# BEAMRobotics/beam_slam

Hardware: AMD Instinct MI355X
Metric: LM iterations/sec + ms/graph-solve, 200KF x 50k-landmark VIO window (higher is better)
Workload: dtype f64; 1 GPU; C2: 200-keyframe x 50000-landmark VIO window; n_obs=400690, n_imu_factors=199, solver_options=vio.yaml:7-17 (<= 10 iterations, tolerances 1.5e-7), max_solver_time lifted, parallelism=single GPU, n_ranks_seen=1

## Files before the change

beam_slam_amd/capi.py:

```python
import ctypes as C

import numpy as np

OK = 0
ERR_INVALID, ERR_DEVICE, ERR_UNSUPPORTED, ERR_NUMERIC = -1, -2, -3, -4

MANIFOLD_EUCLIDEAN, MANIFOLD_QUAT_RIGHT = 0, 1
LOSS_TRIVIAL, LOSS_CAUCHY, LOSS_HUBER = 0, 1, 2

F_REPROJ = 0
F_REPROJ_ONLINE_CALIB = 1
F_IMU_DELTA = 2
F_IMU_PRIOR = 3
F_RELPOSE_EXT = 4
F_RELPOSE = 5
F_ABSPOSE = 6
F_ABS_VEC3 = 7
F_REL_VEC3 = 8
F_GRAVITY = 9
F_IDP_REPROJ = 10
F_IDP_REPROJ_UNARY = 11
F_UNICYCLE = 12
F_NUM_TYPES = 13

# ... 53 lines not shown
        ("iteration", C.c_int32),
        ("step_is_valid", C.c_int32),
        ("step_is_successful", C.c_int32),
        ("reserved0", C.c_int32),
        ("cost", C.c_double),
        ("cost_change", C.c_double),
        ("gradient_max_norm", C.c_double),
        ("gradient_norm", C.c_double),
        ("step_norm", C.c_double),
        ("relative_decrease", C.c_double),
        ("trust_region_radius", C.c_double),
        ("model_cost_change", C.c_double),
    ]


class Camera(C.Structure):
    _fields_ = [
        ("fx", C.c_double), ("fy", C.c_double), ("cx", C.c_double), ("cy", C.c_double),
        ("R_cam_baselink", C.c_double * 9),
        ("t_cam_baselink", C.c_double * 3),
    ]


SYMBOLS = [
    "nidx", "nconst", "nres", "options_default", "options_vio", "create", "create_error", "destroy",
    "last_error", "abi_version", "clear", "set_blocks", "set_values", "set_cameras", "add_factors", "add_factors_indirect", "sync_factors_indirect",
    "add_marginal",
    "finalize", "solve", "get_blocks", "reset_values", "num_iterations_recorded", "get_iteration",
    "evaluate", "num_residuals", "num_parameters_tangent", "tangent_offset", "covariance", "marginalize", "get_marginal",
    "reprojection_errors", "preintegrate", "triangulate", "time_reproj_jacobian_ms", "reproj_jacobian_bytes", "dense_solve", "plan_info",
    "profile_step", "time_eval_ms", "eval_bytes", "bsr_info", "covariance_joint", "update_marginal", "solve_batch", "batch_stats", "set_plan_preference",
    "covariance_requests", "localize_frames", "num_factorizations", "essential_ransac", "absolute_pose_ransac",
    "relative_pose_ransac", "inertial_alignment", "register_scans", "register_scans_error", "backsub_tangent_table",
    "scan_context_describe", "scan_context_match", "scan_context_error",
]

_dp = C.POINTER(C.c_double)
_ip = C.POINTER(C.c_int32)
_bp = C.POINTER(C.c_uint8)

RANSAC_OK, RANSAC_TOO_FEW, RANSAC_NO_MODEL = 0, 1, 2
RANSAC_MAX_MATCHES = 65536
ESSENTIAL_RANSAC_ARGTYPES = [C.c_void_p, C.c_int32, _ip, _dp, _dp, _dp, C.c_double, C.c_double, C.c_int32, C.c_uint64, _bp, _dp, _ip, _ip,
                             _ip, _ip]
ABSOLUTE_POSE_RANSAC_ARGTYPES = [C.c_void_p, C.c_int32, _ip, _dp, _dp, _ip, C.c_double, C.c_double, C.c_int32, C.c_uint64, C.c_int32, _bp,
                                 _dp, _dp, _dp, _ip, _ip, _ip, _ip]
RELATIVE_POSE_RANSAC_ARGTYPES = [C.c_void_p, C.c_int32, _ip, _dp, _dp, _ip, C.c_double, C.c_double, C.c_int32, C.c_uint64, C.c_int32,
                                 C.c_double, C.c_double, _bp, _dp, _dp, _dp, _dp, _bp, _dp, _ip, _ip, _ip, _ip, _ip]
ALIGN_OK, ALIGN_TOO_FEW_FRAMES, ALIGN_BAD_IMU, ALIGN_NOT_EXCITED, ALIGN_RANK_DEFICIENT, ALIGN_SCALE_REJECTED = 0, 1, 2, 3, 4, 5
ALIGN_MIN_EXCITATION, ALIGN_SCALE_MIN, ALIGN_SCALE_MAX, ALIGN_RANK_TOL = 0.25, 0.02, 1.0, 1e-10
INERTIAL_ALIGNMENT_ARGTYPES = [C.c_int, C.c_int32, _ip, _dp, _dp, _dp, _ip, _dp, _dp, _dp, C.c_int32, C.c_double, C.c_int32, C.c_double,
                               C.c_double, C.c_double, _dp, _dp, _dp, _dp, _ip, _dp, _dp, _dp, _dp, _ip]
ICP_MAX_ITERATIONS, ICP_TRANSFORM, ICP_ABS_MSE, ICP_REL_MSE, ICP_TOO_FEW_CORRESPONDENCES = 1, 2, 3, 4, 5
ICP_MAX_CELLS, ICP_MAX_ITER = 1 << 22, 1000
ICP_DEFAULTS = dict(max_corr=1.0, max_iter=50, t_eps=1e-8, fit_eps=1e-2, rotation_threshold=0.99999, rel_mse_eps=1e-5)
REGISTER_SCANS_ARGTYPES = [C.c_int, C.c_int32, _ip, _dp, _ip, _dp, _dp, C.c_double, C.c_int32, C.c_double, C.c_double, C.c_double,
                           C.c_double, _dp, _dp, _dp, _ip, _ip, _ip]
SC_RINGS, SC_SECTORS, SC_MAX_CANDIDATES, SC_MAX_TREE_CANDIDATES, SC_MAX_SCAN_POINTS = 20, 60, 65536, 64, 65535 * 4096
SC_DEFAULTS = dict(lidar_height=2.0, max_radius=80.0, n_tree_candidates=10, search_ratio=0.1, dist_thres=0.3)
SCAN_CONTEXT_DESCRIBE_ARGTYPES = [C.c_int, C.c_int32, _ip, _dp, C.c_int32, _ip, _ip, _dp, C.c_double, C.c_double, _dp, _dp, _dp, _ip]
SCAN_CONTEXT_MATCH_ARGTYPES = [C.c_int, C.c_int32, _ip, _dp, _ip, _dp, C.c_int32, C.c_double, C.c_double, _ip, _dp, _ip, _dp, _dp, _ip]


def _ptr(a, typ):
    return None if a is None else a.ctypes.data_as(typ)


# ... 297 lines not shown
```

beam_slam_amd/csrc/bsgpu_api.cpp:

```cpp
#include <thread>

#include "bsgpu_ctx.h"
#include "bsgpu_env.h"

using namespace bsg;

namespace bsg {
int api_exception(bsgpu_ctx* c) noexcept {
  int code = BSGPU_ERR_INVALID;
  const char* what = "unexpected exception";
  try { throw; }
  catch (const std::bad_alloc&) { code = BSGPU_ERR_DEVICE; what = "out of host memory"; }
  catch (const std::exception& e) { what = e.what(); try { if (c) c->err = std::string("internal error: ") + what; } catch (...) {} return code; }
  catch (...) {}
  try { if (c) c->err = what; } catch (...) {}
  return code;
}
thread_local std::string g_create_error;
int invalidate_keep_values(bsgpu_ctx* c) {
  if (c->finalized && c->d_x && !c->h_x.empty()) {
    HIPCHK(c, hipSetDevice(c->device));
    HIPCHK(c, hipStreamSynchronize(c->stream));
    HIPCHK(c, hipMemcpy(c->h_x.data(), c->d_x, sizeof(double) * c->h_x.size(), hipMemcpyDeviceToHost));
  }
// ... 959 lines not shown
  eval_all(c, c->d_x, true, SC_COST_X);
  (void)hipEventRecord(e0, c->stream);
  for (int i = 0; i < reps; ++i) eval_all(c, c->d_x, true, SC_COST_X);
  (void)hipEventRecord(e1, c->stream);
  if (hipEventSynchronize(e1) != hipSuccess) return -1.0;
  float ms = 0.f;
  (void)hipEventElapsedTime(&ms, e0, e1);
  (void)hipEventDestroy(e0); (void)hipEventDestroy(e1);
  c->spec_J = false;
  return (double)ms / reps;
}
int64_t bsgpu_eval_bytes(const bsgpu_ctx* c) {
  if (!c) return -1;
  static const struct { int idx, consts, res, jcols; } L[BSGPU_F_NUM_TYPES] = {
      {4, 3, 2, 9}, {6, 3, 2, 9}, {10, 287, 15, 30}, {5, 241, 15, 15}, {6, 43, 6, 12}, {4, 43, 6, 12}, {2, 43, 6, 6}, {1, 12, 3, 3},
      {2, 12, 3, 6}, {1, 7, 2, 3}, {6, 6, 2, 13}, {4, 6, 2, 7}, {10, 226, 15, 30}};
  int64_t b = (int64_t)c->vis.n * (c->vis.ja == kJACompact ? 152 : 200) + (int64_t)c->h_x.size() * 8;
  for (int t = 2; t < BSGPU_F_NUM_TYPES && t < kNumInternal; ++t)
    b += (int64_t)c->small[t].n * (4 * L[t].idx + 8 * (L[t].consts + L[t].res + L[t].res * L[t].jcols));
  return b;
}
int bsgpu_bsr_info(bsgpu_ctx* c, int32_t* block_rows, int32_t* nnz_blocks) try {
  if (!c) return BSGPU_ERR_INVALID;
  const int rc = finalize(c);
  if (rc != BSGPU_OK) return rc;
  if (block_rows) *block_rows = c->use_pcg ? c->nbr : 0;
  if (nnz_blocks) *nnz_blocks = c->use_pcg ? c->nblk : 0;
  return BSGPU_OK;
} catch (...) { return api_exception(c); }
int bsgpu_profile_step(bsgpu_ctx* c, const bsgpu_options* o, int32_t reps, double* ms_out, double* work_out) try {
  if (!c) return BSGPU_ERR_INVALID;
  if (!o || !ms_out || reps <= 0) return fail(c, BSGPU_ERR_INVALID, "profile_step: bad argument");
  return profile_step(c, *o, reps, ms_out, work_out);
} catch (...) { return api_exception(c); }
int64_t bsgpu_reproj_jacobian_bytes(const bsgpu_ctx* c) {
  if (!c) return -1;
  return (int64_t)c->vis.n * (c->vis.ja == kJACompact ? 152 : 200) + (int64_t)c->h_x.size() * 8;
}

int bsgpu_dense_solve(int device, int32_t n, const double* A, const double* b, double* x, int32_t max_chains, double* ms_out) try {
  if (n <= 0 || !A || !b || !x) return BSGPU_ERR_INVALID;
  if (hipSetDevice(device) != hipSuccess) return BSGPU_ERR_DEVICE;
  chol_prepare();
  const int T = (n + 63) / 64;
  std::vector<uint8_t> adj((size_t)T * T, 0);
  for (int i = 0; i < n; ++i) for (int j = 0; j < n; ++j) if (A[(size_t)i * n + j] != 0.0) adj[(size_t)(i / 64) * T + j / 64] = 1;
  DensePlan P;
  P.build(n, adj, std::max(1, (int)max_chains), 1, env_shared());
  const int npad = P.npad;
  std::vector<double> hS((size_t)npad * npad, 0.0);
  for (int i = 0; i < n; ++i) for (int j = 0; j < n; ++j) hS[(size_t)P.spos(i) * npad + P.spos(j)] = A[(size_t)i * n + j];
  for (int j = 0; j < n; ++j) hS[(size_t)P.rhs_row * npad + P.spos(j)] = b[j];
  std::vector<uint8_t> real(npad, 0);
  for (int j = 0; j < n; ++j) real[P.spos(j)] = 1;
  for (int i = 0; i < npad; ++i) if (!real[i]) hS[(size_t)i * npad + i] = 1.0;
  double *dS = nullptr, *dLp = nullptr, *dV = nullptr, *dy = nullptr, *dscal = nullptr;
  int *dnreal = nullptr, *drows = nullptr;
  PanelDesc *dpan = nullptr, *dsep = nullptr;
  int *dpot2 = nullptr, *dcb = nullptr, *dce = nullptr, *dsync = nullptr, *dfsync = nullptr, *dtot = nullptr;
  double* dW = nullptr;
  FusedTask* dft = nullptr;
  const bool fused = env_chol_fused() && !P.ftasks.empty();
  hipStream_t s;
  if (hipStreamCreate(&s) != hipSuccess) return BSGPU_ERR_DEVICE;
  auto up = [](const void* src, size_t bytes, void** dst) {
    if (hipMalloc(dst, bytes ? bytes : 8) != hipSuccess) return false;
// ... 74 lines not shown
```

beam_slam_amd/csrc/bsgpu_ctx.h:

```cpp
#pragma once
#include <hip/hip_runtime.h>

#include <algorithm>
#include <chrono>
#include <cmath>
#include <cstdio>
#include <cstdlib>
#include <cstring>
#include <limits>
#include <map>
#include <mutex>
#include <string>
#include <vector>

#include "../../include/bsgpu.h"
#include "bsgpu_internal.h"
#include "dense_plan.h"


namespace bsg {


struct TypeInfo { int nidx, nvar, nconst, m; int amb[10]; };
constexpr int T_REPROJ_DENSE = BSGPU_F_NUM_TYPES;
// ... 118 lines not shown
  double* d_small_part[kNumInternal] = {nullptr};
  double* d_small_part_cand[kNumInternal] = {nullptr};
  double* d_small_part_mcc[kNumInternal] = {nullptr};
  SmallGroup* d_small_groups = nullptr;
  SmallGroup small_factorwise[kNumInternal];
  int n_sa_seg = 0;
  int *d_sa_seg_start = nullptr, *d_sa_seg_ra = nullptr, *d_sa_seg_rb = nullptr;
  int2* d_sa_contrib = nullptr;
  int n_asm_grp = 0;
  AsmGroup* d_asm_grp = nullptr;
  ReduceEntry* d_reduce = nullptr;
  int n_reduce = 0;
  double* d_part_upd = nullptr;
  double* d_gpart = nullptr;
  int n_gpart = 0;
  int n_part_upd = 0;
  int n_upd_blocks = 0;
  bool pre_cleared = false;
  bool upd_in_mcc = false;
  int* d_upd_blocks = nullptr;
  int* d_lm_xoff = nullptr;
  double *d_S = nullptr, *d_grad = nullptr, *d_hdiag = nullptr, *d_scale = nullptr, *d_dcl = nullptr;
  double *d_delta = nullptr, *d_y = nullptr, *d_scal = nullptr, *d_part = nullptr;
  double* h_scal = nullptr;
  double* h_scal_dev = nullptr;
  int dim_model = -1, dim_model_age = 0, dim_model_npose = -1;
  int plan_pref = 0;
  bool spec_dev = false;
  unsigned dec_count = 0;
  double* d_dec = nullptr;
  double spec_lm_radius = 0.0;
  bool spec_cand_arrays = false;
  bool reduce_carried = false;
  bool xpart_stale = false;
  bool spec_dirty = false;
  bool scal_mirrored = false;
  DensePlan plan;
  std::vector<uint8_t> tile_adj;
  int *d_dpos = nullptr, *d_inat = nullptr;
  int *d_nreal = nullptr, *d_rows_flat = nullptr;
  PanelDesc* d_panels = nullptr;
  int *d_bs_desc_chain = nullptr, *d_rows_flat_chain = nullptr, *d_bs_upd = nullptr, *d_bs_upd_rows = nullptr;
  int *d_bs_chain_group = nullptr, *d_bs_grp_nchains = nullptr, *d_bs_grp_nitems = nullptr, *d_bs_items4 = nullptr, *d_bs_tile_updated = nullptr, *d_bs_sync = nullptr, *d_bs_order = nullptr;
  int *d_bs_desc = nullptr, *d_chain_begin = nullptr, *d_chain_end = nullptr, *d_tile_sync = nullptr, *d_touched = nullptr;
  int n_touched = 0;
  int* d_tile_tot = nullptr;
  FusedTask* d_ftasks = nullptr;
  FusedTask* d_ftasks_rows = nullptr; int n_ftasks_rows = 0;
  FusedTask* d_ftasks_bulk = nullptr; int* d_tile_tot_bulk = nullptr; int n_ftasks_bulk = 0;
  FusedTask* d_ftasks_plain = nullptr; int* d_tile_tot_plain = nullptr; int n_ftasks_plain = 0;
  int* d_fsync = nullptr;
  double* d_Vinv = nullptr;
  double* d_Winv = nullptr;
  double* d_Lp = nullptr;
  double* d_ytan = nullptr;
  std::vector<bsgpu_iteration> iters;
  hipGraphExec_t g_first = nullptr, g_accept = nullptr, g_reject = nullptr;
  bool graphs_tried = false, graphs_ok = false, use_graphs = true;
  bsgpu_options graph_opts{};
  double* h_radius = nullptr;
  double* h_pcg = nullptr;
  hipEvent_t pcg_ev[2] = {nullptr, nullptr};
  double* h_pcg_lazy = nullptr;
  bool pcg_check_pending = false;
  int pcg_verdicts_seen = 0;
  hipEvent_t ev_reduce = nullptr;
// ... 99 lines not shown
  std::memcpy(d.R, hc.R_cam_baselink, sizeof(d.R));
  std::memcpy(d.t, hc.t_cam_baselink, sizeof(d.t));
  return d;
}
inline std::vector<DevCamera> dev_cameras(const bsgpu_ctx* c) {
  std::vector<DevCamera> cams;
  cams.reserve(c->cams.size());
  for (const bsgpu_camera& hc : c->cams) cams.push_back(to_dev_camera(hc));
  return cams;
}

#define HIPCHK(c, call)                                                                         \
  do { hipError_t e_ = (call); if (e_ != hipSuccess) return fail(c, BSGPU_ERR_DEVICE, std::string(#call) + ": " + hipGetErrorString(e_)); } while (0)

int materialize_mirror(bsgpu_ctx* c);
int finalize(bsgpu_ctx* c);
int build_bsr(bsgpu_ctx* c);
int build_spcg(bsgpu_ctx* c);
int solve(bsgpu_ctx* c, const bsgpu_options& o, bsgpu_summary& sum);
int check_strategy(bsgpu_ctx* c, const bsgpu_options& o);
void enqueue_fixed_cost(bsgpu_ctx* c, hipStream_t s);
void eval_all(bsgpu_ctx* c, const double* x, bool with_J, int slot, const ReduceRide* red = nullptr);
void assemble(bsgpu_ctx* c, const bsgpu_options& o, double radius, bool new_J, bool first, bool gradient_only = false, bool factor_follows = false,
              const ReduceRide* red = nullptr );
void final_reduce(bsgpu_ctx* c);
int fetch_scalars(bsgpu_ctx* c);
int ensure_vis_src(bsgpu_ctx* c);
void dense_factor(hipStream_t s, const DensePlan& P, const DenseDev& D, double* S, double* scal);
void dense_backsolve(hipStream_t s, const DensePlan& P, const DenseDev& D, double* S, double* y, const int* iperm = nullptr,
                     int n_pose = 0, double* y_tan = nullptr, double* delta = nullptr);
void dense_factor_solve(hipStream_t s, const DensePlan& P, const DenseDev& D, double* S, double* y, double* scal, const int* iperm = nullptr,
                        int n_pose = 0, double* y_tan = nullptr, double* delta = nullptr);
int profile_step(bsgpu_ctx* c, const bsgpu_options& o, int reps, double* ms_out, double* work_out);
bool batch_covers(bsgpu_ctx* c, const bsgpu_options& o);
void batch_stats(int64_t* windows, int64_t* rounds);
bool solve_batched(bsgpu_ctx* const* ctxs, const int* idx, int m, const bsgpu_options* o, int options_stride, bsgpu_summary* s, int* rc);
void batch_forget(const bsgpu_ctx* c);

}
```

beam_slam_amd/csrc/bsgpu_internal.h:

```cpp
#pragma once
#include <hip/hip_runtime.h>
#include <stdint.h>

#include <functional>
#include <cstring>
#include <vector>

#include "dense_plan.h"

struct bsgpu_options;

namespace bsg {

struct DevCamera {
  double fx, fy, cx, cy;
  double R[9];
  double t[3];
};
struct DevLoss {
  int kind;
  int pad;
  double a;
};

// ... 316 lines not shown
void batchargs_small_assemble_seg(BatchArgTable& t, const SmallGroup* groups_dev, int n_seg, const int* seg_start, const int* seg_ra, const int* seg_rb, const int2* contrib,
                                  double* S, int ld, int rhs_row, double* grad, double* hdiag, const int* perm, const SmallGroupSet* fw, int n_fw_units, int n_grp,
                                  const AsmGroup* grp);
void launch_small_assemble_seg_batch(hipStream_t s, const BatchArgTable& t, const BatchDyn* dyn, int list, int n);
bool batchargs_small_mcc(BatchArgTable& t, const SmallGroup* groups, double* const* parts, int n_groups, const double* delta, const UpdateRide* upd, const ZeroStep* zero);
void launch_small_mcc_batch(hipStream_t s, const BatchArgTable& t, const BatchDyn* dyn, int list, int n);
void batchargs_zero_tiles_multi(BatchArgTable& t, const ZeroStep* zs);
void launch_zero_tiles_multi_batch(hipStream_t s, const BatchArgTable& t, const BatchDyn* dyn, int list, int n);
struct MargDev;
bool batchargs_marg_eval(BatchArgTable& t, const MargDev* m, const double* x, double* cost_part);
void launch_marg_eval_batch(hipStream_t s, const BatchArgTable& t, const BatchDyn* dyn, int list, int n, bool with_J);
void batchargs_marg_assemble(BatchArgTable& t, const MargDev* m, double* S, int ld, int rhs_row, double* grad, double* hdiag, const int* perm);
void launch_marg_assemble_batch(hipStream_t s, const BatchArgTable& t, const BatchDyn* dyn, int list, int n);
void batchargs_marg_mcc(BatchArgTable& t, const MargDev* m, const double* delta_tan, double* part);
void launch_marg_mcc_batch(hipStream_t s, const BatchArgTable& t, const BatchDyn* dyn, int list, int n);
struct IdpElim;
void batchargs_idp_landmark(BatchArgTable& t, BatchArgTable& t_view, const IdpElim& e, const SmallGroup& g, int jacobi, double lm_lo, double lm_hi, double* scale, double* dcl, double* grad);
void launch_idp_landmark_batch(hipStream_t s, const BatchArgTable& t, const BatchArgTable& t_view, const BatchDyn* dyn, int list, int n);
void batchargs_idp_pairs(BatchArgTable& t, const IdpElim& e, const SmallGroup& g, double* S, int ld, int rhs_row, double* grad, double* hdiag, const int* perm);
void launch_idp_pairs_batch(hipStream_t s, const BatchArgTable& t, const BatchDyn* dyn, int list, int n);
void batchargs_idp_backsub(BatchArgTable& t, const IdpElim& e, const double* y_pose, double* delta);
void launch_idp_backsub_batch(hipStream_t s, const BatchArgTable& t, const BatchDyn* dyn, int list, int n);
int batchargs_backsolve(BatchArgTable* tabs, const DensePlan& P, const DenseDev& D, double* y, const int* iperm, int n_pose, double* y_tan, double* delta);
void launch_backsolve_batch(hipStream_t s, const BatchArgTable* tabs, const BatchDyn* dyn, const int* n_in_form);
void launch_landmark(hipStream_t s, const Visual& v, int n_pose, const double* radius_ptr, int compute_scale,
                     int compute_dcl, int jacobi, double lm_lo, double lm_hi, double* scale, double* dcl,
                     double* grad, const ZeroStep* zero = nullptr, double radius_val = 0.0, const ReduceRide* red = nullptr );
void launch_pairs(hipStream_t s, const Visual& v, double* S, int ld, int rhs_row, double* grad, double* hdiag, const int* perm,
                  bool grad_only, const SmallGroupSet* small = nullptr, int n_small_units = 0, GoWord go = GoWord());
bool band_available();
void launch_pairs_band(hipStream_t s, const Visual& v, double* S, int ld, int rhs_row, double* grad, double* hdiag, const int* perm,
                       bool grad_only, const SmallGroupSet* small = nullptr, int n_small_units = 0, bool lower_only = false ,
                       GoWord go = GoWord());
int small_assemble_first_set(const SmallGroup* groups, int n_groups, SmallGroupSet* set, int* n_taken);
void launch_small_assemble_set(hipStream_t s, const SmallGroup* groups, int n_groups, double* S, int ld, int rhs_row, double* grad,
                               double* hdiag, const int* perm);
constexpr int kAsmGroupMax = 24;
struct AsmGroup {
  int type, count, m, nv;
  int toff[6];
  int te;
  int pad;
  const double* J;
  const double* r;
  int fac[kAsmGroupMax];
};
bool launch_small_assemble_seg(hipStream_t s, const SmallGroup* groups_dev, int n_seg, const int* seg_start, const int* seg_ra, const int* seg_rb,
                               const int2* contrib, double* S, int ld, int rhs_row, double* grad, double* hdiag, const int* perm,
                               const SmallGroupSet* fw = nullptr, int n_fw_units = 0, int n_grp = 0, const AsmGroup* grp = nullptr,
                               const MargDev* marg = nullptr, const ReduceRide* red = nullptr ,
                               bool* red_carried = nullptr);
void launch_pose_diag(hipStream_t s, int n_pose, double* S, int ld, const double* hdiag, const double* radius_ptr,
                      int compute_scale, int compute_dcl, int jacobi, double lm_lo, double lm_hi, double* scale,
                      double* dcl, int npad, const int* iperm, double radius_val = 0.0 );
void launch_grad_norms(hipStream_t s, int nb, const int* blk_xoff, const int* blk_toff, const unsigned char* blk_size,
                       const unsigned char* blk_manifold, const double* x, const double* grad, double* gpart );
void launch_grad_norms_pose_diag(hipStream_t s, int nb, const int* blk_xoff, const int* blk_toff, const unsigned char* blk_size,
                                 const unsigned char* blk_manifold, const double* x, const double* grad, double* gpart, int n_pose, double* S,
                                 int ld, const double* hdiag, const double* radius_ptr, int compute_scale, int compute_dcl, int jacobi,
                                 double lm_lo, double lm_hi, double* scale, double* dcl, int npad, const int* iperm, double radius_val = 0.0);
struct PanelDesc;
struct FusedTask;
void launch_chol_fused(hipStream_t s, double* S, double* Lp, int ld, const FusedTask* tasks_dev, int n_tasks, const int* tile_tot_dev, const int* nreal_dev,
                       double* Vinv, double* scal, int* sync_dev, double* Winv, int rhs_rows ,
                       const LmDiag& diag = LmDiag(), const GradNormRide& gn = GradNormRide(),
                       bool diag_tasks_in_list = false );
// ... 182 lines not shown
```

beam_slam_amd/csrc/bsgpu_solve.cpp:

```cpp
#include <atomic>

#include <thread>

#include "bsgpu_ctx.h"
#include "bsgpu_env.h"
#include "lm_state.h"

namespace bsg {

void assemble_pcg(bsgpu_ctx* c, const bsgpu_options& o, double radius, bool new_J, bool first) {
  hipStream_t s = c->stream;
  launch_zero4(s, c->d_val, (int64_t)c->nblk * 9, c->d_rhs, c->n_pose, c->d_grad, c->n_pose, c->d_hdiag, c->n_pose);
  for (int t = 2; t < kNumInternal; ++t) launch_bsr_assemble(s, c->small[t], c->d_slots[t], c->d_val);
  launch_bsr_assemble_seg(s, c->d_small_groups, c->n_bsr_seg, c->d_bsr_seg_start, c->d_bsr_seg_slot, c->d_bsr_seg_row, c->d_bsr_contrib, c->d_val, c->d_rhs,
                          c->d_grad, c->d_hdiag);
  launch_bsr_finish_diag(s, c->nbr, c->d_diag_slot, c->d_pair_slot, c->d_val, c->d_hdiag, radius, first ? 1 : 0, new_J ? 1 : 0, o.jacobi_scaling,
                         o.min_lm_diagonal, o.max_lm_diagonal, c->d_scale, c->d_dcl, c->d_Minv);
  if (new_J) {
    launch_grad_norms(s, c->nb, c->d_blk_xoff, c->d_blk_toff, c->d_blk_size, c->d_blk_manifold, c->d_x, c->d_grad, c->d_gpart);
  }
}

static std::atomic<int> g_pcg_persistent_in_flight{0};
void pcg_solve(bsgpu_ctx* c, const bsgpu_options& o) {
// ... 196 lines not shown
  for (size_t i = 0; i < c->marg.size(); ++i) {
    const auto& mc = c->marg[i];
    if (mc.active && (int)i != marg_done) launch_marg_eval(s, mc.dev, x, with_J, cand ? mc.part_cand : mc.part);
  }
  if (with_J) phase_mark(c, BSGPU_PHASE_EVAL_OTHER);
}
bool reduce_can_ride(const bsgpu_ctx* c) {
  static const bool by_event = env_scalars_event(), off = env_reduce_launch();
  return !off && !by_event && !c->use_graphs && !c->use_pcg && !c->prof_events && c->h_scal_dev != nullptr && c->d_reduce_counter != nullptr && c->n_reduce > 0;
}
bool reduce_rides(const bsgpu_ctx* c) {
  static const bool by_event = env_scalars_event(), off = env_reduce_launch();
  static const int merge_mode = env_eval_merge();
  const bool imu_pair = c->small[BSGPU_F_IMU_DELTA].n + c->small[BSGPU_F_IMU_PRIOR].n > 0;
  const bool carrier = imu_pair && merge_mode >= 2 && (c->vis.n > 0 || c->small[BSGPU_F_RELPOSE_EXT].n > 0 || c->small[BSGPU_F_RELPOSE].n > 0);
  return !off && !by_event && !c->use_graphs && !c->use_pcg && !c->prof_events && carrier && c->h_scal_dev != nullptr && c->d_reduce_counter != nullptr &&
         c->n_reduce > 0;
}
void final_reduce(bsgpu_ctx* c) {
  static const bool by_event = env_scalars_event();
  const bool stamp = !c->use_graphs && !by_event && c->h_scal_dev != nullptr && c->d_reduce_counter != nullptr && c->n_reduce > 0;
  if (stamp) c->reduce_seq += 1.0;
  launch_final_reduce(c->stream, c->d_reduce, c->n_reduce, SC_GRAD_NORM2 + 1, c->d_scal, c->h_scal_dev, stamp ? c->d_reduce_counter : nullptr, c->reduce_seq);
  c->scal_mirrored = c->h_scal_dev != nullptr && c->n_reduce > 0;
  c->seq_pending = stamp;
  if (stamp) { c->ev_reduce_pending = false; return; }
  if (c->use_graphs) { c->ev_reduce_pending = false; return; }
  if (!c->ev_reduce && hipEventCreateWithFlags(&c->ev_reduce, hipEventDisableTiming) != hipSuccess) { c->ev_reduce = nullptr; (void)hipGetLastError(); }
  c->ev_reduce_pending = c->scal_mirrored && c->ev_reduce && hipEventRecord(c->ev_reduce, c->stream) == hipSuccess;
}

void assemble(bsgpu_ctx* c, const bsgpu_options& o, double radius, bool new_J, bool first, bool gradient_only, bool factor_follows, const ReduceRide* red) {
  c->reduce_carried = false;
  if (c->use_pcg) { assemble_pcg(c, o, radius, new_J, first); return; }
  hipStream_t s = c->stream;
  ZeroStep zs;
  zs.S = c->d_S; zs.ld = c->npad; zs.tiles = c->d_touched; zs.n_tiles = c->n_touched;
  zs.a = c->d_grad; zs.na = c->n_pose; zs.b = c->d_hdiag; zs.nb = c->n_pose;
  zs.c = new_J ? c->d_scal + SC_GRAD_MAX : c->d_scal + SC_CHOL_FAIL; zs.nc = new_J ? 3 : 1;
  zs.radius_slot = c->use_graphs ? nullptr : c->d_scal + SC_RADIUS; zs.radius = radius;
  const bool dev_decides = red != nullptr && red->lmd.on && red->dec != nullptr && c->vis.n_lm > 0;
  GoWord go;
  if (dev_decides) { zs.radius_slot = nullptr; go.p = red->dec; }
  const bool merged = c->vis.n_lm > 0 && !c->use_graphs;
  const bool cleared = c->pre_cleared && !merged && !c->use_graphs;
  c->pre_cleared = false;
  if (!merged && !cleared) launch_zero_tiles_multi(s, zs.S, zs.ld, zs.tiles, zs.n_tiles, zs.a, zs.na, zs.b, zs.nb, zs.c, zs.nc, zs.radius_slot, zs.radius);
  c->scal_mirrored = false;
  const bool red_in_lm = red != nullptr && c->vis.n_lm > 0;
  if (red_in_lm) zs.nc = 0;
  launch_landmark(s, c->vis, c->n_pose, merged ? nullptr : c->d_scal + SC_RADIUS, first ? 1 : 0, new_J ? 1 : 0, o.jacobi_scaling, o.min_lm_diagonal,
                  o.max_lm_diagonal, c->d_scale, c->d_dcl, c->d_grad, merged ? &zs : nullptr, radius, red_in_lm ? red : nullptr);
  if (red_in_lm) c->reduce_carried = true;
  launch_idp_landmark(s, c->idp, c->small[BSGPU_F_IDP_REPROJ], c->use_graphs ? c->d_scal + SC_RADIUS : nullptr, radius, first ? 1 : 0, new_J ? 1 : 0,
                      o.jacobi_scaling, o.min_lm_diagonal, o.max_lm_diagonal, c->d_scale, c->d_dcl, c->d_grad);
  launch_idp_pairs(s, c->idp, c->small[BSGPU_F_IDP_REPROJ], c->d_S, c->npad, c->plan.rhs_row, c->d_grad, c->d_hdiag, c->d_dpos, gradient_only);
  phase_mark(c, BSGPU_PHASE_LANDMARK);
  int marg_done = -1;
  {
    SmallGroupSet set;
    int taken = 0, units = 0;
    const bool band = c->vis.n_band_units > 0;
    if (c->vis.n_seg > 0 || band) units = small_assemble_first_set(c->small_factorwise + 2, kNumInternal - 2, &set, &taken);
    if (units == 0) taken = 0;
    const bool lower_only = factor_follows && !gradient_only && !c->use_spcg && !c->use_pcg && c->dense_ok && c->d_ftasks && c->d_fsync && c->d_tile_tot && c->d_Winv;
    if (band) launch_pairs_band(s, c->vis, c->d_S, c->npad, c->plan.rhs_row, c->d_grad, c->d_hdiag, c->d_dpos, gradient_only, units > 0 ? &set : nullptr, units, lower_only, go);
    launch_pairs(s, c->vis, c->d_S, c->npad, c->plan.rhs_row, c->d_grad, c->d_hdiag, c->d_dpos, gradient_only, (units > 0 && !band) ? &set : nullptr, band ? 0 : units, go);
    if (c->calib.on) launch_calib_border(s, c->vis, c->calib, c->d_S, c->npad, c->plan.rhs_row, c->d_grad, c->d_hdiag, c->d_dpos, gradient_only);
// ... 274 lines not shown
    c->spec_J = false;
    c->prof_events = ev.data() + (size_t)r * ne;
    (void)hipEventRecord(c->prof_events[0], c->stream);
    enqueue_step(c, o, STEP_ACCEPT, radius);
    c->prof_events = nullptr;
  }
  HIPCHK(c, hipStreamSynchronize(c->stream));
  c->scal_mirrored = false; c->ev_reduce_pending = false; c->spec_J = false;
  for (int p = 0; p < BSGPU_PHASE_NUM; ++p) ms_out[p] = 0.0;
  for (int r = 0; r < reps; ++r)
    for (int p = 0; p < BSGPU_PHASE_NUM; ++p) {
      float ms = 0.f;
      (void)hipEventElapsedTime(&ms, ev[(size_t)r * ne + p], ev[(size_t)r * ne + p + 1]);
      ms_out[p] += (double)ms / reps;
    }
  for (auto& e : ev) (void)hipEventDestroy(e);
  if (work_out) {
    const double n = (double)c->vis.n, ne_ = (double)c->vis.n_elim, nl = (double)c->vis.n_lm, nent = (double)c->vis.n_ent;
    for (int p = 0; p < BSGPU_PHASE_NUM; ++p) work_out[p] = 0.0;
    const double ja_b = 8.0 * c->vis.ja;
    work_out[BSGPU_PHASE_EVAL_REPROJ] = n * (104.0 + ja_b) + 8.0 * (double)c->h_x.size();
    const double cr = c->vis.no_cr ? 0.0 : 64.0;
    work_out[BSGPU_PHASE_LANDMARK] = ne_ * (48.0 + 16.0 + cr) + nl * (72.0 + 24.0 + 48.0 + 4.0) + 32768.0 * (double)c->n_touched + 16.0 * (double)c->n_pose;
    work_out[BSGPU_PHASE_PAIRS] = ne_ * (ja_b + (c->vis.no_cr ? 48.0 : 64.0) + (c->vis.n_band_units > 0 ? 16.0 : 0.0)) + nent * 8.0 + (c->vis.no_cr ? nl * 72.0 : 0.0);
    work_out[BSGPU_PHASE_FACTOR] = c->plan.fused_flops;
    work_out[BSGPU_PHASE_BACKSUB] = n * (ja_b + 48.0 + 16.0) + ne_ * cr + nl * 72.0;
    work_out[BSGPU_PHASE_CANDIDATE] = n * 40.0 + 3.0 * 8.0 * (double)c->h_x.size();
  }
  HIPCHK(c, hipMemcpyAsync(c->d_x, c->d_x0, sizeof(double) * c->h_x.size(), hipMemcpyDeviceToDevice, c->stream));
  HIPCHK(c, hipStreamSynchronize(c->stream));
  return BSGPU_OK;
}

bool same_graph_options(const bsgpu_options& a, const bsgpu_options& b) {
  return a.jacobi_scaling == b.jacobi_scaling && a.min_lm_diagonal == b.min_lm_diagonal && a.max_lm_diagonal == b.max_lm_diagonal &&
         a.linear_solver_type == b.linear_solver_type;
}

void build_graphs(bsgpu_ctx* c, const bsgpu_options& o) {
  if (c->graphs_tried && same_graph_options(o, c->graph_opts)) return;
  c->destroy_graphs();
  c->graphs_tried = true;
  c->graph_opts = o;
  if (!c->use_graphs || c->use_pcg || c->use_spcg) return;
  hipGraphExec_t* execs[3] = {&c->g_first, &c->g_accept, &c->g_reject};
  for (int kind = 0; kind < 3; ++kind) {
    hipGraph_t graph = nullptr;
    if (hipStreamBeginCapture(c->stream, hipStreamCaptureModeThreadLocal) != hipSuccess) { (void)hipGetLastError(); return; }
    enqueue_step(c, o, kind, 1.0);
    if (hipStreamEndCapture(c->stream, &graph) != hipSuccess || !graph) { (void)hipGetLastError(); c->destroy_graphs(); c->graphs_tried = true; return; }
    const hipError_t e = hipGraphInstantiate(execs[kind], graph, nullptr, nullptr, 0);
    (void)hipGraphDestroy(graph);
    if (e != hipSuccess) { (void)hipGetLastError(); c->destroy_graphs(); c->graphs_tried = true; return; }
  }
  c->graphs_ok = true;
  if (env_timing()) fprintf(stderr, "[bsgpu] LM step captured as hipGraphs\n");
}

void run_step(bsgpu_ctx* c, const bsgpu_options& o, int kind, double radius, bool gradient_only = false, double radius_ahead = 0.0, const LmDecide* lmd = nullptr) {
  if (c->use_graphs) {
    *c->h_radius = radius;
    (void)hipMemcpyAsync(c->d_scal + SC_RADIUS, c->h_radius, sizeof(double), hipMemcpyHostToDevice, c->stream);
  }
  if (c->graphs_ok && !gradient_only) {
    hipGraphExec_t g = kind == STEP_FIRST ? c->g_first : kind == STEP_ACCEPT ? c->g_accept : c->g_reject;
    if (hipGraphLaunch(g, c->stream) == hipSuccess) return;
// ... 311 lines not shown
```

beam_slam_amd/gpu.py:

```python
import ctypes
import os

from . import capi

_HERE = os.path.dirname(os.path.abspath(__file__))
LIB_PATH = os.path.join(_HERE, "csrc", "libbsgpu.so")
_LIB = None


class GpuLibraryMissing(RuntimeError):
    pass


def lib():
    global _LIB
    if _LIB is None:
        if not os.path.exists(LIB_PATH):
            raise GpuLibraryMissing(
                f"{LIB_PATH} is missing: build it with `python -c 'import __graft_entry__ as g; g.build()'` "
                "(hipcc --offload-arch=gfx950).  beam_slam_amd has no CPU fallback.")
        _LIB = ctypes.CDLL(LIB_PATH)
        _LIB.bsgpu_time_reproj_jacobian_ms.restype = ctypes.c_double
        _LIB.bsgpu_time_reproj_jacobian_ms.argtypes = [ctypes.c_void_p, ctypes.c_int32]
        _LIB.bsgpu_time_eval_ms.restype = ctypes.c_double
# ... 294 lines not shown

    def eval_bytes(self):
        return lib().bsgpu_eval_bytes(self._ctx)

    def bsr_info(self):
        a, b = ctypes.c_int32(0), ctypes.c_int32(0)
        self._chk(lib().bsgpu_bsr_info(ctypes.c_void_p(self._ctx), ctypes.byref(a), ctypes.byref(b)))
        return a.value, b.value

    PHASES = ("eval_reproj", "eval_other", "landmark", "pairs", "assemble_other", "factor", "backsolve", "backsub", "candidate")

    def profile_step(self, options=None, reps=10):
        import numpy as np
        opt = options if options is not None else self.options_default()
        ms, work = np.zeros(len(self.PHASES)), np.zeros(len(self.PHASES))
        fn = lib().bsgpu_profile_step
        fn.argtypes = [ctypes.c_void_p, ctypes.c_void_p, ctypes.c_int32, ctypes.c_void_p, ctypes.c_void_p]
        self._chk(fn(self._ctx, ctypes.byref(opt), int(reps), ms.ctypes.data, work.ctypes.data))
        return {name: (float(ms[i]), float(work[i])) for i, name in enumerate(self.PHASES)}

    def set_plan_preference(self, throughput):
        fn = lib().bsgpu_set_plan_preference
        fn.argtypes = [ctypes.c_void_p, ctypes.c_int32]
        self._chk(fn(self._ctx, 1 if throughput else 0))

    def plan_info(self):
        a, b, c = ctypes.c_int32(0), ctypes.c_int32(0), ctypes.c_int32(0)
        self.finalize()
        lib().bsgpu_plan_info(ctypes.c_void_p(self._ctx), ctypes.byref(a), ctypes.byref(b), ctypes.byref(c))
        return a.value, b.value, c.value

    def reproj_jacobian_bytes(self):
        return lib().bsgpu_reproj_jacobian_bytes(self._ctx)
```

include/bsgpu.h:

```cpp
#ifndef BSGPU_H_
#define BSGPU_H_

#include <stdint.h>

#ifdef __cplusplus
extern "C" {
#endif

#define BSGPU_ABI_VERSION 1

enum {
  BSGPU_OK = 0,
  BSGPU_ERR_INVALID = -1,
  BSGPU_ERR_DEVICE = -2,
  BSGPU_ERR_UNSUPPORTED = -3,
  BSGPU_ERR_NUMERIC = -4
};

enum {
  BSGPU_MANIFOLD_EUCLIDEAN = 0,
  BSGPU_MANIFOLD_QUAT_RIGHT = 1
};

enum {
// ... 228 lines not shown
                           double* E, int32_t* n_inliers, int32_t* n_iters, int32_t* best_sample, int32_t* status);

int bsgpu_absolute_pose_ransac(bsgpu_ctx* ctx, int32_t n_frames, const int32_t* obs_start, const double* pixels,
                               const double* points, const int32_t* camera, double prob, double threshold_px,
                               int32_t max_iters, uint64_t seed, int32_t truncate_pixels, uint8_t* mask,
                               double* q_out, double* p_out, double* T_cam_world, int32_t* n_inliers,
                               int32_t* n_iters, int32_t* best_sample, int32_t* status);

int bsgpu_relative_pose_ransac(bsgpu_ctx* ctx, int32_t n_sets, const int32_t* match_start, const double* px_first,
                               const double* px_last, const int32_t* camera, double prob, double threshold_px,
                               int32_t max_iters, uint64_t seed, int32_t truncate_pixels, double validate_px,
                               double min_inlier_ratio, uint8_t* mask, double* T_last_first, double* q_out, double* p_out,
                               double* points, uint8_t* valid_mask, double* inlier_ratio, int32_t* pair_valid,
                               int32_t* n_inliers, int32_t* n_iters, int32_t* best_sample, int32_t* status);

double bsgpu_time_reproj_jacobian_ms(bsgpu_ctx* ctx, int32_t reps);
double bsgpu_time_eval_ms(bsgpu_ctx* ctx, int32_t reps);
int64_t bsgpu_eval_bytes(const bsgpu_ctx* ctx);
int bsgpu_bsr_info(bsgpu_ctx* ctx, int32_t* block_rows, int32_t* nnz_blocks);
int64_t bsgpu_reproj_jacobian_bytes(const bsgpu_ctx* ctx);
enum {
  BSGPU_PHASE_EVAL_REPROJ = 0,
  BSGPU_PHASE_EVAL_OTHER = 1,
  BSGPU_PHASE_LANDMARK = 2,
  BSGPU_PHASE_PAIRS = 3,
  BSGPU_PHASE_ASSEMBLE_OTHER = 4,
  BSGPU_PHASE_FACTOR = 5,
  BSGPU_PHASE_BACKSOLVE = 6,
  BSGPU_PHASE_BACKSUB = 7,
  BSGPU_PHASE_CANDIDATE = 8,
  BSGPU_PHASE_NUM = 9
};
int bsgpu_profile_step(bsgpu_ctx* ctx, const bsgpu_options* options, int32_t reps, double* ms_out, double* work_out);

int bsgpu_dense_solve(int device, int32_t n, const double* A, const double* b, double* x,
                      int32_t max_chains, double* ms_out);
int bsgpu_plan_info(const bsgpu_ctx* ctx, int32_t* n_chains, int32_t* n_steps, int32_t* n_tiles);
enum { BSGPU_PLAN_LATENCY = 0, BSGPU_PLAN_THROUGHPUT = 1 };
int bsgpu_set_plan_preference(bsgpu_ctx* ctx, int32_t preference);

#ifdef __cplusplus
}
#endif
#endif
```

Measured before the change: 3837 LM iterations/s.

## Add a dedicated visual gradient kernel for gradient-only assembly

Adds a gradient-only assembly path that skips building the Schur complement. A new kernel accumulates landmark and camera-pose gradients from the reprojection Jacobians, using LDS atomics per camera and riding the small factors in the same launch. The path only runs when graphs are off and several other conditions hold, and a new gradient_step API exercises it. In the normal LM solve with graphs enabled the new path is likely skipped, so it may not change timed iterations.

```diff
diff --git a/beam_slam_amd/capi.py b/beam_slam_amd/capi.py
--- a/beam_slam_amd/capi.py
+++ b/beam_slam_amd/capi.py
@@ -109,7 +109,7 @@
     "profile_step", "time_eval_ms", "eval_bytes", "bsr_info", "covariance_joint", "update_marginal", "solve_batch", "batch_stats", "set_plan_preference",
     "covariance_requests", "localize_frames", "num_factorizations", "essential_ransac", "absolute_pose_ransac",
     "relative_pose_ransac", "inertial_alignment", "register_scans", "register_scans_error", "backsub_tangent_table",
-    "scan_context_describe", "scan_context_match", "scan_context_error",
+    "scan_context_describe", "scan_context_match", "scan_context_error", "gradient_step",
 ]
 
 _dp = C.POINTER(C.c_double)
diff --git a/beam_slam_amd/csrc/bsgpu_api.cpp b/beam_slam_amd/csrc/bsgpu_api.cpp
--- a/beam_slam_amd/csrc/bsgpu_api.cpp
+++ b/beam_slam_amd/csrc/bsgpu_api.cpp
@@ -1015,6 +1015,11 @@
   if (!c) return BSGPU_ERR_INVALID;
   if (!o || !ms_out || reps <= 0) return fail(c, BSGPU_ERR_INVALID, "profile_step: bad argument");
   return profile_step(c, *o, reps, ms_out, work_out);
+} catch (...) { return api_exception(c); }
+int bsgpu_gradient_step(bsgpu_ctx* c, const bsgpu_options* o, double* gradient, int32_t* used_gradient_launch) try {
+  if (!c) return BSGPU_ERR_INVALID;
+  if (!o || !gradient) return fail(c, BSGPU_ERR_INVALID, "gradient_step: bad argument");
+  return gradient_step(c, *o, gradient, used_gradient_launch);
 } catch (...) { return api_exception(c); }
 int64_t bsgpu_reproj_jacobian_bytes(const bsgpu_ctx* c) {
   if (!c) return -1;
diff --git a/beam_slam_amd/csrc/bsgpu_ctx.h b/beam_slam_amd/csrc/bsgpu_ctx.h
--- a/beam_slam_amd/csrc/bsgpu_ctx.h
+++ b/beam_slam_amd/csrc/bsgpu_ctx.h
@@ -174,6 +174,7 @@
   double spec_lm_radius = 0.0;
   bool spec_cand_arrays = false;
   bool reduce_carried = false;
+  bool grad_launch_used = false;
   bool xpart_stale = false;
   bool spec_dirty = false;
   bool scal_mirrored = false;
@@ -339,6 +340,7 @@
 void dense_factor_solve(hipStream_t s, const DensePlan& P, const DenseDev& D, double* S, double* y, double* scal, const int* iperm = nullptr,
                         int n_pose = 0, double* y_tan = nullptr, double* delta = nullptr);
 int profile_step(bsgpu_ctx* c, const bsgpu_options& o, int reps, double* ms_out, double* work_out);
+int gradient_step(bsgpu_ctx* c, const bsgpu_options& o, double* gradient, int32_t* used_gradient_launch);
 bool batch_covers(bsgpu_ctx* c, const bsgpu_options& o);
 void batch_stats(int64_t* windows, int64_t* rounds);
 bool solve_batched(bsgpu_ctx* const* ctxs, const int* idx, int m, const bsgpu_options* o, int options_stride, bsgpu_summary* s, int* rc);
diff --git a/beam_slam_amd/csrc/bsgpu_internal.h b/beam_slam_amd/csrc/bsgpu_internal.h
--- a/beam_slam_amd/csrc/bsgpu_internal.h
+++ b/beam_slam_amd/csrc/bsgpu_internal.h
@@ -372,6 +372,8 @@
 void launch_pairs_band(hipStream_t s, const Visual& v, double* S, int ld, int rhs_row, double* grad, double* hdiag, const int* perm,
                        bool grad_only, const SmallGroupSet* small = nullptr, int n_small_units = 0, bool lower_only = false ,
                        GoWord go = GoWord());
+bool visual_gradient_available(const Visual& v);
+void launch_visual_gradient(hipStream_t s, const Visual& v, int n_pose, double* grad, const SmallGroupSet* small = nullptr, int n_small_units = 0);
 int small_assemble_first_set(const SmallGroup* groups, int n_groups, SmallGroupSet* set, int* n_taken);
 void launch_small_assemble_set(hipStream_t s, const SmallGroup* groups, int n_groups, double* S, int ld, int rhs_row, double* grad,
                                double* hdiag, const int* perm);
diff --git a/beam_slam_amd/csrc/bsgpu_solve.cpp b/beam_slam_amd/csrc/bsgpu_solve.cpp
--- a/beam_slam_amd/csrc/bsgpu_solve.cpp
+++ b/beam_slam_amd/csrc/bsgpu_solve.cpp
@@ -252,8 +252,30 @@
 
 void assemble(bsgpu_ctx* c, const bsgpu_options& o, double radius, bool new_J, bool first, bool gradient_only, bool factor_follows, const ReduceRide* red) {
   c->reduce_carried = false;
+  c->grad_launch_used = false;
   if (c->use_pcg) { assemble_pcg(c, o, radius, new_J, first); return; }
   hipStream_t s = c->stream;
+  if (gradient_only && new_J && !first && red == nullptr) {
+    SmallGroupSet set;
+    int taken = 0;
+    const int units = small_assemble_first_set(c->small + 2, kNumInternal - 2, &set, &taken);
+    bool plain = !c->use_graphs && !c->use_spcg && !c->calib.on && c->idp.n_lm == 0 && c->small[BSGPU_F_IDP_REPROJ].n == 0 &&
+                 c->small[BSGPU_F_IDP_REPROJ_UNARY].n == 0 && visual_gradient_available(c->vis);
+    for (int t = 2 + taken; t < kNumInternal; ++t) plain = plain && c->small[t].n == 0;
+    for (const auto& mc : c->marg) plain = plain && !mc.active;
+    if (plain) {
+      c->pre_cleared = false; c->scal_mirrored = false; c->diag_in_chol = false;
+      c->lm_diag = LmDiag(); c->gn_ride = GradNormRide();
+      c->grad_launch_used = true;
+      launch_zero_tiles_multi(s, c->d_S, c->npad, c->d_touched, 0, c->d_grad, c->n_pose, nullptr, 0, c->d_scal + SC_GRAD_MAX, 3, c->d_scal + SC_RADIUS, radius);
+      launch_visual_gradient(s, c->vis, c->n_pose, c->d_grad, units > 0 ? &set : nullptr, units);
+      phase_mark(c, BSGPU_PHASE_LANDMARK);
+      phase_mark(c, BSGPU_PHASE_PAIRS);
+      launch_grad_norms(s, c->nb, c->d_blk_xoff, c->d_blk_toff, c->d_blk_size, c->d_blk_manifold, c->d_x, c->d_grad, c->d_gpart);
+      phase_mark(c, BSGPU_PHASE_ASSEMBLE_OTHER);
+      return;
+    }
+  }
   ZeroStep zs;
   zs.S = c->d_S; zs.ld = c->npad; zs.tiles = c->d_touched; zs.n_tiles = c->n_touched;
   zs.a = c->d_grad; zs.na = c->n_pose; zs.b = c->d_hdiag; zs.nb = c->n_pose;
@@ -594,6 +616,28 @@
   return BSGPU_OK;
 }
 
+int gradient_step(bsgpu_ctx* c, const bsgpu_options& o, double* gradient, int32_t* used_gradient_launch) {
+  int rc = finalize(c);
+  if (rc != BSGPU_OK) return rc;
+  if (!c->dense_ok) return fail(c, BSGPU_ERR_UNSUPPORTED, "gradient_step: dense Schur path only");
+  HIPCHK(c, hipSetDevice(c->device));
+  c->use_pcg = false; c->use_spcg = false;
+  c->spec_J = false; c->spec_cand_arrays = false; c->spec_lm_radius = 0.0; c->spec_dirty = false; c->spec_dev = false;
+  const double radius = o.initial_trust_region_radius;
+  if (c->use_graphs) {
+    *c->h_radius = radius;
+    (void)hipMemcpyAsync(c->d_scal + SC_RADIUS, c->h_radius, sizeof(double), hipMemcpyHostToDevice, c->stream);
+  }
+  eval_all(c, c->d_x, true, SC_COST_X);
+  assemble(c, o, radius, true, true);
+  assemble(c, o, radius, true, false, true, true);
+  if (used_gradient_launch) *used_gradient_launch = c->grad_launch_used ? 1 : 0;
+  HIPCHK(c, hipMemcpyAsync(gradient, c->d_grad, sizeof(double) * (size_t)c->n_tan, hipMemcpyDeviceToHost, c->stream));
+  HIPCHK(c, hipStreamSynchronize(c->stream));
+  c->scal_mirrored = false; c->ev_reduce_pending = false; c->pre_cleared = false;
+  return BSGPU_OK;
+}
+
 bool same_graph_options(const bsgpu_options& a, const bsgpu_options& b) {
   return a.jacobi_scaling == b.jacobi_scaling && a.min_lm_diagonal == b.min_lm_diagonal && a.max_lm_diagonal == b.max_lm_diagonal &&
          a.linear_solver_type == b.linear_solver_type;
diff --git a/beam_slam_amd/csrc/k_grad.hip b/beam_slam_amd/csrc/k_grad.hip
--- /dev/null
+++ b/beam_slam_amd/csrc/k_grad.hip
@@ -0,0 +1,116 @@
+#include <cstring>
+
+#include "bsgpu_device.h"
+
+namespace bsg {
+
+constexpr int kGradMaxWgs = 1024;
+constexpr size_t kGradMaxLds = 48 * 1024;
+
+BSG_DEV void small_gradient_unit(const SmallGroupSet& set, int unit, int lane, int n_pose, double* __restrict__ grad) {
+  if (unit >= set.first[set.n]) return;
+  int gi = 0;
+  while (gi + 1 < set.n && unit >= set.first[gi + 1]) ++gi;
+  const SmallGroup& g = set.g[gi];
+  const int f = unit - set.first[gi];
+  if (!g.active[f]) return;
+  const int m = g.m, tw = 3 * g.nv;
+  const int wcut = 3 * (g.nv - 1) + g.w_last;
+  const double* J = g.J + (size_t)f * m * tw;
+  const double* r = g.r + (size_t)f * m;
+  for (int a = lane; a < wcut; a += 64) {
+    const int t = g.toff[(size_t)f * g.nv + a / 3];
+    if (t < 0 || t + a % 3 >= n_pose) continue;
+    double gs = 0.0;
+    for (int k = 0; k < m; ++k) gs += J[k * tw + a] * r[k];
+    atomicAdd(&grad[t + a % 3], gs);
+  }
+}
+
+template <bool COMPACT>
+__global__ __launch_bounds__(256) void visual_gradient_kernel(int n_lm, const int* __restrict__ lm_order, const int* __restrict__ lm_start, const double* __restrict__ JA, const double* __restrict__ JB,
+                                                              const double2* __restrict__ r, const int* __restrict__ cam_pose, int n_cam_pose,
+                                                              const int* __restrict__ cp_tq, const int* __restrict__ cp_tp, int n_pose, double* __restrict__ grad,
+                                                              int lm_blocks, int blocks_per_wg, int n_rider_wgs, SmallGroupSet small) {
+  if ((int)blockIdx.x < n_rider_wgs) {
+    small_gradient_unit(small, (int)blockIdx.x * 4 + (int)(threadIdx.x >> 6), (int)(threadIdx.x & 63), n_pose, grad);
+    return;
+  }
+  extern __shared__ __attribute__((aligned(16))) double cam_tab[];
+  const int n_tab = 6 * n_cam_pose;
+  for (int i = threadIdx.x; i < n_tab; i += 256) cam_tab[i] = 0.0;
+  __syncthreads();
+  const int wg = (int)blockIdx.x - n_rider_wgs;
+  const int b0 = wg * blocks_per_wg, b1 = min(b0 + blocks_per_wg, lm_blocks);
+  constexpr int kJA = COMPACT ? kJACompact : kJAStride;
+  for (int blk = b0; blk < b1; ++blk) {
+    const int gid = blk * 256 + threadIdx.x;
+    const int li = gid >> 3, sub = gid & 7;
+    const bool valid = li < n_lm;
+    const int l = valid ? lm_order[li] : 0;
+    int beg = 0, end = 0;
+    if (valid) { beg = lm_start[l]; end = lm_start[l + 1]; }
+    double g0 = 0, g1 = 0, g2 = 0;
+    for (int f = beg + sub; f < end; f += 8) {
+      const double2* Jf2 = reinterpret_cast<const double2*>(JB + (size_t)f * 6);
+      const double2* Af2 = reinterpret_cast<const double2*>(JA + (size_t)f * kJA);
+      const double2 rf = r[f];
+      const double2 ja = Jf2[0], jb = Jf2[1], jc = Jf2[2];
+      const double2 a0 = Af2[0], a1 = Af2[1], a2 = Af2[2];
+      const int cam = cam_pose[f];
+      const double x0 = ja.x, x1 = ja.y, x2 = jb.x, y0 = jb.y, y1 = jc.x, y2 = jc.y;
+      g0 += x0 * rf.x + y0 * rf.y; g1 += x1 * rf.x + y1 * rf.y; g2 += x2 * rf.x + y2 * rf.y;
+      double A0[6], A1[6];
+      if (COMPACT) {
+        A0[0] = a0.x; A0[1] = a0.y; A0[2] = a1.x; A0[3] = -x0; A0[4] = -x1; A0[5] = -x2;
+        A1[0] = a1.y; A1[1] = a2.x; A1[2] = a2.y; A1[3] = -y0; A1[4] = -y1; A1[5] = -y2;
+      } else {
+        const double2 a3 = Af2[COMPACT ? 0 : 3], a4 = Af2[COMPACT ? 0 : 4], a5 = Af2[COMPACT ? 0 : 5];
+        A0[0] = a0.x; A0[1] = a0.y; A0[2] = a1.x; A0[3] = a1.y; A0[4] = a2.x; A0[5] = a2.y;
+        A1[0] = a3.x; A1[1] = a3.y; A1[2] = a4.x; A1[3] = a4.y; A1[4] = a5.x; A1[5] = a5.y;
+      }
+      if (cam >= 0 && cam < n_cam_pose) {
+        double* t = cam_tab + 6 * cam;
+#pragma unroll
+        for (int m = 0; m < 6; ++m) atomicAdd(&t[m], fma(A0[m], rf.x, A1[m] * rf.y));
+      }
+    }
+#pragma unroll
+    for (int o = 4; o > 0; o >>= 1) { g0 += __shfl_xor(g0, o, 8); g1 += __shfl_xor(g1, o, 8); g2 += __shfl_xor(g2, o, 8); }
+    if (valid && sub == 0) {
+      const int to = n_pose + 3 * l;
+      grad[to] = g0; grad[to + 1] = g1; grad[to + 2] = g2;
+    }
+  }
+  __syncthreads();
+  for (int i = threadIdx.x; i < n_tab; i += 256) {
+    const double v = cam_tab[i];
+    if (v == 0.0) continue;
+    const int cam = i / 6, m = i - 6 * cam;
+    const int t = m < 3 ? cp_tq[cam] : cp_tp[cam];
+    if (t < 0) continue;
+    const int ti = t + (m < 3 ? m : m - 3);
+    if (ti < n_pose) atomicAdd(&grad[ti], v);
+  }
+}
+
+bool visual_gradient_available(const Visual& v) {
+  return v.n_lm > 0 && v.no_cr && v.n == v.n_elim && v.n_seg == 0 && v.cam_pose != nullptr && v.band_lm_id != nullptr && v.n_band_lm == v.n_lm && (v.ja == kJACompact || v.ja == kJAStride) &&
+         sizeof(double) * 6 * (size_t)v.n_cam_pose <= kGradMaxLds;
+}
+void launch_visual_gradient(hipStream_t s, const Visual& v, int n_pose, double* grad, const SmallGroupSet* small, int n_small_units) {
+  static const SmallGroupSet none = [] { SmallGroupSet e; std::memset(&e, 0, sizeof(e)); return e; }();
+  const int lm_blocks = (v.n_lm * 8 + 255) / 256;
+  const int per = (lm_blocks + kGradMaxWgs - 1) / kGradMaxWgs;
+  const int wgs = (lm_blocks + per - 1) / per;
+  const int riders = small ? (n_small_units + 3) / 4 : 0;
+  const size_t lds = sizeof(double) * 6 * (size_t)v.n_cam_pose;
+  if (v.ja == kJACompact)
+    hipLaunchKernelGGL(visual_gradient_kernel<true>, dim3(riders + wgs), dim3(256), lds, s, v.n_lm, v.band_lm_id, v.lm_start, v.J, v.JB, v.r, v.cam_pose, v.n_cam_pose, v.cp_tq, v.cp_tp,
+                       n_pose, grad, lm_blocks, per, riders, small ? *small : none);
+  else
+    hipLaunchKernelGGL(visual_gradient_kernel<false>, dim3(riders + wgs), dim3(256), lds, s, v.n_lm, v.band_lm_id, v.lm_start, v.J, v.JB, v.r, v.cam_pose, v.n_cam_pose, v.cp_tq, v.cp_tp,
+                       n_pose, grad, lm_blocks, per, riders, small ? *small : none);
+}
+
+}
diff --git a/beam_slam_amd/gpu.py b/beam_slam_amd/gpu.py
--- a/beam_slam_amd/gpu.py
+++ b/beam_slam_amd/gpu.py
@@ -350,3 +350,14 @@
 
     def reproj_jacobian_bytes(self):
         return lib().bsgpu_reproj_jacobian_bytes(self._ctx)
+
+    def gradient_step(self, opt=None):
+        import numpy as np
+        self.finalize()
+        fn = lib().bsgpu_gradient_step
+        fn.argtypes = [ctypes.c_void_p, ctypes.c_void_p, ctypes.c_void_p, ctypes.POINTER(ctypes.c_int32)]
+        opt = opt if opt is not None else self.options_default()
+        g = np.zeros(self.num_parameters_tangent())
+        used = ctypes.c_int32(0)
+        self._chk(fn(self._ctx, ctypes.byref(opt), g.ctypes.data, ctypes.byref(used)))
+        return g, bool(used.value)
diff --git a/include/bsgpu.h b/include/bsgpu.h
--- a/include/bsgpu.h
+++ b/include/bsgpu.h
@@ -284,6 +284,7 @@
   BSGPU_PHASE_NUM = 9
 };
 int bsgpu_profile_step(bsgpu_ctx* ctx, const bsgpu_options* options, int32_t reps, double* ms_out, double* work_out);
+int bsgpu_gradient_step(bsgpu_ctx* ctx, const bsgpu_options* options, double* gradient, int32_t* used_gradient_launch);
 
 int bsgpu_dense_solve(int device, int32_t n, const double* A, const double* b, double* x,
                       int32_t max_chains, double* ms_out);
```

After: 3876 LM iterations/s, median of 4. 1.0% higher.
